# noway/nzcb-circom

Measured on AMD Instinct MI355X. Metric: PLONK proofs/sec for nzcp_live (~2^21 constraints) at 1/2/4/8 MI355X, higher is better.
Workload: dtype u32 limbs: BN254 Fr/Fq Montgomery, 8x32-bit and 9x29-bit (MSM, NTT twiddles, quotient); 1 GPU; nzcp_live fullProve: NZCPPubIdentity(1,351,0,4,2,4) witness on the GPU (600560 signals) + PLONK proof, n=2^21, nPublic=3, 2970 inputs; domain_size=2097152, n_public=3, n_constraints=1785813, n_vars=1782570, n_additions=1182010, proofs_per_gpu=140, total_proofs=140, parallelism=batch-shard x1 (no collective), proofs_in_flight_per_gpu=5

## Files before the change

### nzcb-circom_amd/csrc/msm.h

```cpp
#pragma once
#include <vector>

#include "common.h"
#include "ec.h"
#include "f29.h"

namespace nzcb {

struct MsmBaseTable {
  DevBuf<G1Affine> q;
  size_t n = 0, stride = 0;
  int c = 0, nw = 0;
  bool mont_folded = false;
  bool sparse = false;
  void build(const G1Affine* bases, size_t n, int c, hipStream_t st, bool fold_mont = false);
};

int fixed_base_window();
int lagrange_window();
bool lagrange_sparse();

struct MsmScratch {
  size_t max_points = 0;
  int max_lsets = 1;
  DevBuf<uint32_t> offsets;
  DevBuf<uint32_t> sorted;
  DevBuf<uint32_t> keys_in, keys_out, vals_in;
  DevBuf<uint8_t> sort_tmp;
  size_t sort_tmp_bytes = 0;
  DevBuf<uint32_t> bin_counts, vals_mid;
  DevBuf<uint32_t> lo_seg;
  DevBuf<G1xyzz> buckets;
  DevBuf<G1xyzz> carry_own;
  DevBuf<G1xyzz> carry_cont;
  DevBuf<Xyzz29> buckets29, carry_own29, carry_cont29;
  DevBuf<uint32_t> large;
  DevBuf<uint32_t> large_off;
  DevBuf<Xyzz29> large_part;
  DevBuf<Xyzz29> rowp29, colp29, lines29;
  DevBuf<G1xyzz> seg_tot;
  DevBuf<G1xyzz> seg_run;
  DevBuf<G1xyzz> parts;
  DevBuf<G1xyzz> win;
  G1xyzz* host_win = nullptr;
  uint32_t* host_total = nullptr;
  size_t host_win_cap = 0;
  int cur_c = 0, cur_nsets = 0, cur_nbits = 0, cur_seglen = 0;
  bool cur_fixed = false, cur_sparse = false;
  int cur_a = 0, cur_hb = 0;
  int cur_msets = 1;
  size_t cur_n = 0;
  uint32_t cur_nkeys = 0;
  bool prof = false, prof_phases = false;
  double prof_ms = 0;
  double phase_ms[7] = {0, 0, 0, 0, 0, 0, 0};
  double host_ms = 0;
  double enqueue_ms = 0;
  double sort_host_ms = 0;
  uint64_t prof_launches = 0, prof_points = 0, prof_entries = 0;
  hipEvent_t ev[8] = {nullptr, nullptr, nullptr, nullptr, nullptr, nullptr, nullptr, nullptr};
  hipEvent_t done = nullptr;
  void init(size_t max_points, bool fixed_base = false, int lagrange_sets = 1, bool generic = true);
  ~MsmScratch();
};

int msm_window_bits(size_t n);

void msm_enqueue(MsmScratch& sc, const G1Affine* bases, const Fr* scalars, size_t n, bool scalars_mont,
                 hipStream_t st, const MsmBaseTable* table = nullptr);
G1xyzz msm_finish(MsmScratch& sc, hipStream_t st);
void msm_enqueue_sets(MsmScratch& sc, const Fr* const* scalars, int sets, size_t n, bool scalars_mont,
                      hipStream_t st, const MsmBaseTable* table);
void msm_finish_sets(MsmScratch& sc, hipStream_t st, G1xyzz* out);

inline G1xyzz msm(MsmScratch& sc, const G1Affine* bases, const Fr* scalars, size_t n, bool mont, hipStream_t st,
                  const MsmBaseTable* table = nullptr) {
  msm_enqueue(sc, bases, scalars, n, mont, st, table);
  return msm_finish(sc, st);
}

G1Affine xyzz_to_affine(const G1xyzz& p);

}
```

### nzcb-circom_amd/csrc/msm.hip

```cpp
#include "msm.h"

#include "f29.h"

#include <chrono>
#include <cstdlib>
#include <type_traits>
#include <rocprim/rocprim.hpp>
#include <rocprofiler-sdk-roctx/roctx.h>

namespace nzcb {

static constexpr int kMsmThreads = 256;

#ifndef NZ_TAIL_PRIO
#define NZ_TAIL_PRIO 0
#endif
__device__ __forceinline__ void tail_prio() {
  if constexpr (NZ_TAIL_PRIO > 0) __builtin_amdgcn_s_setprio(NZ_TAIL_PRIO);
}

using SortConfig = rocprim::radix_sort_config<
    rocprim::default_config, rocprim::default_config,
    rocprim::radix_sort_onesweep_config<rocprim::kernel_config<1024, 16>, rocprim::kernel_config<1024, 16>, 10,
                                        rocprim::block_radix_rank_algorithm::match>>;
// ... 17 lines not shown
static constexpr uint32_t kSeqSpan = 64;
static constexpr uint32_t kSeqSpan29 = 16;
static constexpr int kLargeBlocks = 32;
static constexpr int kLargePieceBlocks = 128;
static constexpr int kLargeFinalBlocks = 128;

static constexpr uint32_t kDynThreads = 1u << 18;
static constexpr uint32_t kDynMin = 8;
static constexpr uint32_t kSeqSpanSparse = 3;
static constexpr int kSparsePieceBlocks = 2048;
static constexpr int kSparseFinalBlocks = 512;
__host__ __device__ __forceinline__ uint32_t dyn_chunk(uint32_t m) {
  const uint32_t c = (m + kDynThreads - 1) / kDynThreads;
  return c < kDynMin ? kDynMin : c > kChunk ? kChunk : c;
}
static size_t dyn_threads_bound(size_t entries) {
  const size_t lo = std::min<size_t>(kDynThreads, (entries + kDynMin - 1) / kDynMin);
  return std::max<size_t>(lo, (entries + kChunk - 1) / kChunk);
}

static constexpr int kFbWindow = 20;
int fixed_base_window() {
  static const int c = [] {
    const char* e = std::getenv("NZCB_FB_WINDOW");
    const int v = e ? std::atoi(e) : kFbWindow;
    return (v >= 16 && v <= 20) ? v : kFbWindow;
  }();
  return c;
}

#ifndef NZ_LAGRANGE_WINDOW
#define NZ_LAGRANGE_WINDOW 17
#endif
int lagrange_window() { return NZ_LAGRANGE_WINDOW; }
bool lagrange_sparse() {
  static const bool v = [] {
    const char* e = std::getenv("NZCB_SPARSE");
    return e && std::atoi(e) != 0;
  }();
  return v;
}

int msm_window_bits(size_t n) {
  if (n >= (size_t(1) << 18)) return 16;
  int lg = ilog2(n ? n : 1);
  int c = lg - 3;
  if (c < 4) c = 4;
  if (c > 16) c = 16;
  return c;
}

static inline int num_windows(int c) { return (255 + c - 1) / c; }

template <int C, class F>
__device__ __forceinline__ void for_each_digit(const Fr& s, F&& f) {
  constexpr int NW = (255 + C - 1) / C;
  constexpr uint32_t MASK = (1u << C) - 1u;
  constexpr uint32_t HALF = 1u << (C - 1);
  uint32_t carry = 0;
#pragma unroll
  for (int w = 0; w < NW; w++) {
    const int bit = w * C;
    const int limb = bit >> 5;
    const int sh = bit & 31;
    uint64_t x = s.v[limb];
    if (limb + 1 < 8) x |= (uint64_t)s.v[limb + 1] << 32;
    uint32_t d = ((uint32_t)(x >> sh) & MASK) + carry;
    if (d > HALF) {
      uint32_t mag = (MASK + 1u) - d;
      if (mag) f(w, mag - 1u, 1u);
      carry = 1;
    } else {
      if (d) f(w, d - 1u, 0u);
      carry = 0;
    }
  }
}

#ifdef NZCB_MSM_STATS
template <class F>
static void for_each_digit_host(const Fr& s, int C, F&& f) {
  const int NW = (255 + C - 1) / C;
  const uint32_t MASK = (1u << C) - 1u, HALF = 1u << (C - 1);
  uint32_t carry = 0;
  for (int w = 0; w < NW; w++) {
    const int bit = w * C, limb = bit >> 5, sh = bit & 31;
    uint64_t x = s.v[limb];
    if (limb + 1 < 8) x |= (uint64_t)s.v[limb + 1] << 32;
    uint32_t d = ((uint32_t)(x >> sh) & MASK) + carry;
    if (d > HALF) {
      uint32_t mag = (MASK + 1u) - d;
      if (mag) f(w, mag - 1u, 1u);
      carry = 1;
    } else {
      if (d) f(w, d - 1u, 0u);
      carry = 0;
    }
  }
}
#endif

template <int C>
__global__ void __launch_bounds__(kMsmThreads)
msm_keys_kernel(const Fr* __restrict__ scalars, size_t n, int mont, uint32_t* __restrict__ keys,
                uint32_t* __restrict__ vals) {
  constexpr int NW = (255 + C - 1) / C;
  constexpr uint32_t NB = 1u << (C - 1);
  constexpr uint32_t SENTINEL = NW * NB;
  for (size_t i = (size_t)blockIdx.x * blockDim.x + threadIdx.x; i < n; i += (size_t)gridDim.x * blockDim.x) {
    Fr s = scalars[i];
    if (mont) s = from_mont_fr29(s);
    uint32_t k[NW];
#pragma unroll
    for (int w = 0; w < NW; w++) k[w] = SENTINEL;
    uint32_t sg[NW];
#pragma unroll
    for (int w = 0; w < NW; w++) sg[w] = 0;
    for_each_digit<C>(s, [&](int w, uint32_t b, uint32_t sign) {
      k[w] = (uint32_t)w * NB + b;
      sg[w] = sign << 31;
    });
#pragma unroll
    for (int w = 0; w < NW; w++) {
      keys[(size_t)w * n + i] = k[w];
      vals[(size_t)w * n + i] = (uint32_t)i | sg[w];
    }
  }
}

static constexpr int kBinThreads = 256;
static constexpr int kBinPer = 2;
static constexpr uint32_t kTileScalars = kBinThreads * kBinPer;
static constexpr int kLoThreads = 512;

static constexpr int kDigMont = 1;
static constexpr int kDigMinForm = 2;

__device__ __forceinline__ uint32_t scalar_min_form(Fr& s) {
  constexpr uint32_t H[8] = {0xf8000000u, 0xa1f0fac9u, 0x3cdcb848u, 0x9419f424u,
                             0x40c0ac2eu, 0xdc2822dbu, 0x7098d014u, 0x18322739u};
  bool gt = false, eq = true, lt_r = false, eq_r = true;
#pragma unroll
  for (int l = 7; l >= 0; l--) {
    gt = gt || (eq && s.v[l] > H[l]);
    eq = eq && s.v[l] == H[l];
    lt_r = lt_r || (eq_r && s.v[l] < FrParams::P[l]);
    eq_r = eq_r && s.v[l] == FrParams::P[l];
  }
  if (!(gt && lt_r)) return 0u;
  s = neg(s);
  return 1u;
}

template <int C, int NW>
__device__ __forceinline__ uint32_t bin_entries(const Fr* __restrict__ scalars, size_t i, int mont, size_t stride,
                                                uint32_t (&kk)[NW], uint32_t (&vv)[NW]) {
  Fr s = scalars[i];
  if (mont & kDigMont) s = from_mont_fr29(s);
  const uint32_t flip = (mont & kDigMinForm) ? scalar_min_form(s) : 0u;
  uint32_t live = 0;
#pragma unroll
  for (int w = 0; w < NW; w++) {
    kk[w] = 0;
    vv[w] = 0;
  }
  for_each_digit<C>(s, [&](int w, uint32_t b, uint32_t sign) {
    kk[w] = b;
    vv[w] = (uint32_t)((size_t)w * stride + i) | ((sign ^ flip) << 31);
    live |= 1u << w;
  });
  return live;
}

template <int KB> struct BinKeys {
  static constexpr int LO = KB - 8 > 8 ? KB - 8 : 8;
  using Lo = typename std::conditional<LO <= 8, uint8_t, uint16_t>::type;
  using Full = typename std::conditional<KB <= 16, uint16_t, uint32_t>::type;
};

static constexpr int kMaxSets = 3;
struct BinSets {
  const Fr* p[kMaxSets];
  uint32_t tps;
  uint32_t nb;
};

template <int C, int KB>
__global__ void __launch_bounds__(kBinThreads)
msm_bin_hist_kernel(BinSets sets, size_t n, int mont, uint32_t* __restrict__ counts, uint32_t ntiles) {
  constexpr int NW = (255 + C - 1) / C;
  constexpr int LO = BinKeys<KB>::LO;
  __shared__ uint32_t h[256];
  h[threadIdx.x] = 0;
  __syncthreads();
  const uint32_t set = blockIdx.x / sets.tps, lt = blockIdx.x - set * sets.tps;
  const Fr* __restrict__ scalars = sets.p[set];
  const uint32_t kbase = set * sets.nb;
#pragma unroll
  for (int j = 0; j < kBinPer; j++) {
    const size_t i = (size_t)lt * kTileScalars + (size_t)j * kBinThreads + threadIdx.x;
    if (i < n) {
      uint32_t kk[NW], vv[NW];
      const uint32_t live = bin_entries<C, NW>(scalars, i, mont, 0, kk, vv);
#pragma unroll
      for (int w = 0; w < NW; w++)
        if ((live >> w) & 1u) atomicAdd(&h[(kk[w] + kbase) >> LO], 1u);
    }
  }
  __syncthreads();
  counts[(size_t)threadIdx.x * ntiles + blockIdx.x] = h[threadIdx.x];
}

__device__ __forceinline__ uint32_t wave_incl_scan(uint32_t v) {
  const int lane = threadIdx.x & 63;
#pragma unroll
  for (int off = 1; off < 64; off <<= 1) {
    const uint32_t u = __shfl_up(v, off, 64);
    if (lane >= off) v += u;
  }
  return v;
}

__device__ __forceinline__ uint32_t scan256_excl(uint32_t v, uint32_t* wsum4, uint32_t& total) {
  const uint32_t inc = wave_incl_scan(threadIdx.x < 256 ? v : 0u);
  if (threadIdx.x < 256 && (threadIdx.x & 63) == 63) wsum4[threadIdx.x >> 6] = inc;
  __syncthreads();
  uint32_t off = 0;
  for (int w = 0; w < (int)(threadIdx.x >> 6) && w < 4; w++) off += wsum4[w];
  total = wsum4[0] + wsum4[1] + wsum4[2] + wsum4[3];
  __syncthreads();
  return threadIdx.x < 256 ? off + inc - v : 0u;
}

__global__ void __launch_bounds__(256)
msm_bin_rowscan_kernel(uint32_t* __restrict__ counts, uint32_t ntiles, uint32_t* __restrict__ tail) {
  __shared__ uint32_t wsum[4];
  uint32_t* row = counts + (size_t)blockIdx.x * ntiles;
  uint32_t carry = 0;
  for (uint32_t c0 = 0; c0 < ntiles; c0 += 256) {
    const uint32_t t = c0 + threadIdx.x;
    const uint32_t v = t < ntiles ? row[t] : 0u;
    uint32_t tot;
    const uint32_t ex = scan256_excl(v, wsum, tot);
    if (t < ntiles) row[t] = carry + ex;
    carry += tot;
  }
  if (threadIdx.x == 0) tail[blockIdx.x] = carry;
}

template <int C, int KB>
__global__ void __launch_bounds__(kBinThreads)
msm_bin_scatter_kernel(BinSets sets, size_t n, int mont, size_t stride, const uint32_t* __restrict__ counts,
                       uint32_t ntiles, typename BinKeys<KB>::Lo* __restrict__ lo2, uint32_t* __restrict__ vals2) {
  constexpr int NW = (255 + C - 1) / C;
  constexpr int TE = kTileScalars * NW;
  constexpr int LO = BinKeys<KB>::LO;
  __shared__ uint32_t lcount[256], lstart[256], gbase[256];
  __shared__ uint32_t lval[TE];
  __shared__ typename BinKeys<KB>::Full lkey[TE];
  const uint32_t set = blockIdx.x / sets.tps, lt = blockIdx.x - set * sets.tps;
  const Fr* __restrict__ scalars = sets.p[set];
  const uint32_t kbase = set * sets.nb;
  __shared__ uint32_t wsum[4];
  const uint32_t* tail = counts + (size_t)256 * ntiles;
  {
    uint32_t tot;
    const uint32_t st = scan256_excl(tail[threadIdx.x], wsum, tot);
    gbase[threadIdx.x] = st + counts[(size_t)threadIdx.x * ntiles + blockIdx.x];
    lcount[threadIdx.x] = 0;
  }
  __syncthreads();
  uint32_t kk[kBinPer][NW], vv[kBinPer][NW], rk[kBinPer][NW], live[kBinPer];
#pragma unroll
  for (int j = 0; j < kBinPer; j++) {
    const size_t i = (size_t)lt * kTileScalars + (size_t)j * kBinThreads + threadIdx.x;
    live[j] = 0;
    if (i < n) {
      live[j] = bin_entries<C, NW>(scalars, i, mont, stride, kk[j], vv[j]);
#pragma unroll
      for (int w = 0; w < NW; w++) {
        kk[j][w] += kbase;
        if ((live[j] >> w) & 1u) rk[j][w] = atomicAdd(&lcount[kk[j][w] >> LO], 1u);
      }
    }
  }
  __syncthreads();
  uint32_t total;
  {
    lstart[threadIdx.x] = scan256_excl(lcount[threadIdx.x], wsum, total);
  }
  __syncthreads();
#pragma unroll
  for (int j = 0; j < kBinPer; j++) {
#pragma unroll
    for (int w = 0; w < NW; w++) {
      if ((live[j] >> w) & 1u) {
        const uint32_t q = lstart[kk[j][w] >> LO] + rk[j][w];
        lkey[q] = (typename BinKeys<KB>::Full)kk[j][w];
        lval[q] = vv[j][w];
      }
    }
  }
  __syncthreads();
  for (uint32_t q = threadIdx.x; q < total; q += kBinThreads) {
    const uint32_t key = lkey[q], hb = key >> LO;
    const uint32_t pos = gbase[hb] + (q - lstart[hb]);
    lo2[pos] = (typename BinKeys<KB>::Lo)(key & ((1u << LO) - 1u));
    vals2[pos] = lval[q];
  }
}

template <int NT>
__device__ __forceinline__ uint32_t block_scan_excl(uint32_t* a, uint32_t count, uint32_t* wsum) {
  const uint32_t per = (count + NT - 1) / NT;
  const uint32_t b = threadIdx.x * per;
  uint32_t loc = 0;
  for (uint32_t i = 0; i < per; i++)
    if (b + i < count) loc += a[b + i];
  const uint32_t inc = wave_incl_scan(loc);
  if ((threadIdx.x & 63) == 63) wsum[threadIdx.x >> 6] = inc;
  __syncthreads();
  uint32_t off = 0, tot = 0;
#pragma unroll
  for (int w = 0; w < NT / 64; w++) {
    if (w < (int)(threadIdx.x >> 6)) off += wsum[w];
    tot += wsum[w];
  }
  uint32_t run = off + inc - loc;
  for (uint32_t i = 0; i < per; i++)
    if (b + i < count) {
      const uint32_t v = a[b + i];
      a[b + i] = run;
      run += v;
    }
  __syncthreads();
  return tot;
}

static constexpr uint32_t kLoSeg = 32768;
static constexpr uint32_t kLoU = 8;

__device__ __forceinline__ void lo_regions(const uint32_t* __restrict__ tail, uint32_t* wsum, uint32_t* rs,
                                           uint32_t* rf) {
  const uint32_t t = threadIdx.x;
  const uint32_t cnt = t < 256 ? tail[t] : 0u;
  uint32_t tot, nitems;
  const uint32_t st = scan256_excl(cnt, wsum, tot);
  const uint32_t f = scan256_excl((cnt + kLoSeg - 1) / kLoSeg, wsum, nitems);
  if (t < 256) {
    rs[t] = st;
    rf[t] = f;
  }
  if (t == 0) rf[256] = nitems;
  __syncthreads();
}

__device__ __forceinline__ uint32_t lo_region_of(const uint32_t* rf, uint32_t item) {
  uint32_t lo = 0, hi = 256;
  while (hi - lo > 1) {
    const uint32_t mid = (lo + hi) >> 1;
    if (rf[mid] <= item) lo = mid; else hi = mid;
  }
  return lo;
}

template <int LO>
__global__ void __launch_bounds__(kLoThreads)
msm_lo_count_kernel(const typename std::conditional<LO <= 8, uint8_t, uint16_t>::type* __restrict__ lo2,
                    const uint32_t* __restrict__ counts, uint32_t ntiles, uint32_t* __restrict__ segoff) {
  constexpr uint32_t NL = 1u << LO;
  __shared__ uint32_t h[NL], wsum[kLoThreads / 64], rs[256], rf[257];
  lo_regions(counts + (size_t)256 * ntiles, wsum, rs, rf);
  const uint32_t item = blockIdx.x;
  if (item >= rf[256]) return;
  const uint32_t r = lo_region_of(rf, item);
  const uint32_t* tail = counts + (size_t)256 * ntiles;
  const uint32_t s = rs[r] + (item - rf[r]) * kLoSeg;
  const uint32_t e = min(rs[r] + tail[r], s + kLoSeg);
  for (uint32_t i = threadIdx.x; i < NL; i += kLoThreads) h[i] = 0;
  __syncthreads();
  for (uint32_t p0 = s; p0 < e; p0 += kLoU * kLoThreads) {
    uint32_t k8[kLoU];
#pragma unroll
    for (uint32_t u = 0; u < kLoU; u++) {
      const uint32_t q = p0 + u * kLoThreads + threadIdx.x;
      k8[u] = q < e ? (uint32_t)lo2[q] : NL;
    }
#pragma unroll
    for (uint32_t u = 0; u < kLoU; u++)
      if (k8[u] < NL) atomicAdd(&h[k8[u]], 1u);
  }
  __syncthreads();
  for (uint32_t i = threadIdx.x; i < NL; i += kLoThreads) segoff[(size_t)item * NL + i] = h[i];
}

template <int LO>
__global__ void __launch_bounds__(kLoThreads)
msm_lo_scan_kernel(const uint32_t* __restrict__ counts, uint32_t ntiles, uint32_t* __restrict__ segoff,
                   uint32_t nkeys, uint32_t* __restrict__ offsets, uint32_t* __restrict__ large) {
  constexpr uint32_t NL = 1u << LO;
  __shared__ uint32_t h[NL], wsum[kLoThreads / 64], rs[256], rf[257];
  const uint32_t* tail = counts + (size_t)256 * ntiles;
  lo_regions(tail, wsum, rs, rf);
  const uint32_t hb = blockIdx.x;
  const uint32_t f0 = rf[hb], ns = rf[hb + 1] - f0, s = rs[hb];
  for (uint32_t i = threadIdx.x; i < NL; i += kLoThreads) {
    uint32_t run = 0;
    for (uint32_t g = 0; g < ns; g++) {
      uint32_t* c = segoff + (size_t)(f0 + g) * NL + i;
      const uint32_t v = *c;
      *c = run;
      run += v;
    }
    h[i] = run;
  }
  __syncthreads();
  block_scan_excl<kLoThreads>(h, NL, wsum);
  for (uint32_t i = threadIdx.x; i < NL; i += kLoThreads) {
    const uint32_t base = s + h[i];
    const uint32_t key = (hb << LO) | i;
    if (key < nkeys) offsets[key] = base;
    for (uint32_t g = 0; g < ns; g++) segoff[(size_t)(f0 + g) * NL + i] += base;
  }
  if (hb == 255 && threadIdx.x == 0) offsets[nkeys] = s + tail[255];
  if (hb == 0 && threadIdx.x == 0) large[0] = 0;
}

template <int LO, int NT = kLoThreads, uint32_t U = kLoU>
__global__ void __launch_bounds__(NT)
msm_lo_scatter_kernel(const typename std::conditional<LO <= 8, uint8_t, uint16_t>::type* __restrict__ lo2,
                      const uint32_t* __restrict__ vals2, const uint32_t* __restrict__ counts, uint32_t ntiles,
                      const uint32_t* __restrict__ segoff, uint32_t* __restrict__ sorted) {
  using Lo = typename std::conditional<LO <= 8, uint8_t, uint16_t>::type;
  constexpr uint32_t NL = 1u << LO;
  constexpr uint32_t kLoThreads = NT, kLoU = U;
  __shared__ uint32_t h[NL], lcnt[NL], lst[NL];
  __shared__ uint32_t wsum[kLoThreads / 64], rs[256], rf[257];
  __shared__ uint32_t lv[kLoU * kLoThreads];
  __shared__ Lo lk[kLoU * kLoThreads];
  lo_regions(counts + (size_t)256 * ntiles, wsum, rs, rf);
  const uint32_t item = blockIdx.x;
  if (item >= rf[256]) return;
  const uint32_t r = lo_region_of(rf, item);
  const uint32_t* tail = counts + (size_t)256 * ntiles;
  const uint32_t s = rs[r] + (item - rf[r]) * kLoSeg;
  const uint32_t e = min(rs[r] + tail[r], s + kLoSeg);
  for (uint32_t i = threadIdx.x; i < NL; i += kLoThreads) h[i] = segoff[(size_t)item * NL + i];
  for (uint32_t p0 = s; p0 < e; p0 += kLoU * kLoThreads) {
    uint32_t k8[kLoU], v8[kLoU], r8[kLoU];
    for (uint32_t i = threadIdx.x; i < NL; i += kLoThreads) lcnt[i] = 0;
    __syncthreads();
#pragma unroll
// ... 663 lines not shown
    if (s == 0 && blockIdx.y == 0 && total_out) host_put(total_out, *entries);
    host_put_done();
  }
}

__global__ void __launch_bounds__(kMsmThreads)
msm_table_kernel(const G1Affine* __restrict__ bases, size_t n, size_t stride, int c, int nw, Fq k261, int fold,
                 Fr kinv, G1Affine* __restrict__ q) {
  const size_t i = (size_t)blockIdx.x * blockDim.x + threadIdx.x;
  if (i >= n) return;
  const G1Affine P = bases[i];
  if (P.is_inf()) {
    for (int w = 0; w < nw; w++) q[(size_t)w * stride + i] = P;
    return;
  }
  G1xyzz acc = xyzz_from_affine(P);
  if (fold) {
    acc = G1xyzz::inf();
    for (int b = 253; b >= 0; b--) {
      acc = xyzz_dbl(acc);
      if ((kinv.v[b >> 5] >> (b & 31)) & 1u) acc = xyzz_add_affine(acc, P.x, P.y);
    }
  }
  for (int w = 0; w < nw; w++) {
    if (w)
      for (int k = 0; k < c; k++) acc = xyzz_dbl(acc);
    const Fq ti = inverse(acc.ZZ * acc.ZZZ);
    G1Affine r;
    r.x = acc.X * (acc.ZZZ * ti) * k261;
    r.y = acc.Y * (acc.ZZ * ti) * k261;
    q[(size_t)w * stride + i] = r;
  }
}

void MsmBaseTable::build(const G1Affine* bases, size_t npts, int cbits, hipStream_t st, bool fold_mont) {
  n = npts;
  mont_folded = fold_mont;
  stride = npts;
  c = cbits;
  nw = num_windows(c);
  if ((size_t)nw * stride >= (size_t(1) << 31)) throw Error(NZCB_ERR_ARG, "msm table too large for 31-bit indices");
  q.alloc((size_t)nw * stride);
  Fq thirty_two = Fq::zero();
  thirty_two.v[0] = 32;
  const Fq k261 = to_mont(thirty_two);
  Fr one_raw = Fr::zero();
  one_raw.v[0] = 1;
  const Fr kinv = from_mont(one_raw);
  hipLaunchKernelGGL(msm_table_kernel, dim3(grid_for(n, kMsmThreads, 1u << 30)), dim3(kMsmThreads), 0, st, bases, n,
                     stride, c, nw, k261, fold_mont ? 1 : 0, kinv, q.p);
  NZ_HIP(hipGetLastError());
}

static void lmark(const char* what) {
  static const bool on = std::getenv("NZCB_MARK_LAUNCHES") != nullptr;
  if (on) roctxMarkA(what);
}

static size_t lo_items_bound(size_t entries) { return 256 + entries / kLoSeg + 1; }

struct MsmPlan {
  int c, nw, nsets, seglen, nseg, nbits, nslots, nparts;
  int lb, a, hb, ltiles, htiles;
  int msets;
  uint32_t nb, nkeys;
  size_t entries;
};

static MsmPlan make_plan(size_t n, const MsmBaseTable* t, int msets = 1) {
  MsmPlan p;
  p.c = t ? t->c : msm_window_bits(n);
  p.nw = num_windows(p.c);
  p.nsets = t ? 1 : p.nw;
  p.msets = t ? msets : 1;
  p.nb = 1u << (p.c - 1);
  p.nkeys = p.nb * (uint32_t)p.nsets * (uint32_t)p.msets;
  p.seglen = (int)(p.nb < (uint32_t)kSegLen ? p.nb : kSegLen);
  p.nseg = (int)(p.nb / p.seglen);
  p.nbits = 0;
  while ((1 << p.nbits) < p.nseg) p.nbits++;
  p.nslots = p.nbits + 1;
  p.nparts = (p.nseg + kSumThreads * kSumPer - 1) / (kSumThreads * kSumPer);
  p.lb = p.c - 1;
  p.a = (p.lb + 1) / 2;
  p.hb = p.lb - p.a;
  p.ltiles = (1 << p.a) / kTileSide;
  p.htiles = (1 << p.hb) / kTileSide;
  p.entries = n * (size_t)p.nw * (size_t)p.msets;
  return p;
}

void MsmScratch::init(size_t maxp, bool fixed_base, int lagrange_sets, bool generic) {
  if (lagrange_sets < 1 || lagrange_sets > kMaxSets) throw Error(NZCB_ERR_ARG, "msm scratch: 1..3 Lagrange sets");
  if (!fixed_base) generic = true;
  max_points = maxp;
  max_lsets = lagrange_sets;
  size_t max_entries = 0, max_keys = 0, max_seg = 0, max_slots = 0, max_parts = 0, max_tiles = 0, max_lines = 0;
  auto fit = [&](const MsmPlan& p) {
    max_entries = std::max(max_entries, p.entries);
    max_keys = std::max(max_keys, (size_t)p.nkeys);
    if (p.nsets == 1) {
      max_slots = std::max(max_slots, (size_t)(p.lb + 1) * p.msets);
      max_tiles = std::max(max_tiles, (size_t)p.nb / kTileSide * p.msets);
      max_lines = std::max(max_lines, (((size_t)1 << p.hb) + ((size_t)1 << p.a)) * p.msets);
    } else {
      max_seg = std::max(max_seg, (size_t)p.nseg * p.nsets);
      max_slots = std::max(max_slots, (size_t)p.nslots * p.nsets);
      max_parts = std::max(max_parts, (size_t)p.nslots * p.nsets * p.nparts);
    }
  };
  for (size_t n = 1;; n <<= 1) {
    size_t m = n < maxp ? n : maxp;
    fit(make_plan(m, nullptr));
    if (m == maxp) break;
  }
  MsmPlan fp{};
  if (fixed_base) {
    MsmBaseTable t;
    t.c = fixed_base_window();
    fp = make_plan(maxp, &t);
    fit(fp);
    t.c = lagrange_window();
    const MsmPlan lp = make_plan(maxp, &t, lagrange_sets);
    fit(lp);
    if (lp.entries > fp.entries) fp = lp;
  }
  const size_t ge = generic ? max_entries : 1;
  offsets.alloc(max_keys + 1);
  sorted.alloc(max_entries);
  keys_in.alloc(ge);
  keys_out.alloc(max_entries);
  vals_in.alloc(ge);
  sort_tmp_bytes = 0;
  if (generic) {
    radix_sort(nullptr, sort_tmp_bytes, keys_in.p, keys_out.p, vals_in.p, sorted.p, max_entries, 21, nullptr);
  }
  sort_tmp.alloc(sort_tmp_bytes + 16);
  const size_t nthreads = std::max((max_entries + kChunk - 1) / kChunk, dyn_threads_bound(max_entries)) + 1;
  buckets.alloc(generic ? max_keys : 1);
  carry_own.alloc(generic ? nthreads : 1);
  carry_cont.alloc(generic ? nthreads : 1);
  large.alloc(max_keys + 1);
  if (fixed_base) {
    buckets29.alloc(max_keys);
    large_off.alloc(max_keys + 2);
    large_part.alloc(nthreads / kPieceCarries + max_keys + 1);
    carry_own29.alloc(nthreads);
    carry_cont29.alloc(nthreads);
    rowp29.alloc(max_tiles);
    colp29.alloc(max_tiles);
    lines29.alloc(max_lines);
    bin_counts.alloc((size_t)256 * ((maxp + kTileScalars - 1) / kTileScalars) * lagrange_sets + 256);
    vals_mid.alloc(max_entries);
    lo_seg.alloc(lo_items_bound(max_entries) * ((size_t)1 << BinKeys<19>::LO));
  }
  seg_tot.alloc(max_seg && generic ? max_seg : 1);
  seg_run.alloc(max_seg && generic ? max_seg : 1);
  parts.alloc(max_parts && generic ? max_parts : 1);
  win.alloc(max_slots);
  host_win_cap = max_slots;
  NZ_HIP(hipHostMalloc((void**)&host_win, (max_slots + 1) * sizeof(G1xyzz), hipHostMallocCoherent));
  host_total = (uint32_t*)(host_win + max_slots);
}

MsmScratch::~MsmScratch() {
  if (host_win) (void)hipHostFree(host_win);
  if (done) (void)hipEventDestroy(done);
  for (auto& e : ev)
    if (e) (void)hipEventDestroy(e);
}

static void keys_dispatch(int c, const Fr* scalars, size_t n, int mont, MsmScratch& sc, hipStream_t st) {
  auto launch = [&](auto cc) {
    constexpr int C = decltype(cc)::value;
    hipLaunchKernelGGL(msm_keys_kernel<C>, dim3(grid_for(n, kMsmThreads, 1u << 30)), dim3(kMsmThreads), 0, st,
                       scalars, n, mont, sc.keys_in.p, sc.vals_in.p);
  };
  switch (c) {
#define NZ_CASE(K) case K: launch(std::integral_constant<int, K>()); break;
    NZ_CASE(4) NZ_CASE(5) NZ_CASE(6) NZ_CASE(7) NZ_CASE(8) NZ_CASE(9) NZ_CASE(10) NZ_CASE(11) NZ_CASE(12)
    NZ_CASE(13) NZ_CASE(14) NZ_CASE(15) NZ_CASE(16)
#undef NZ_CASE
    default: throw Error(NZCB_ERR_INTERNAL, "bad msm window");
  }
  NZ_HIP(hipGetLastError());
}

G1Affine xyzz_to_affine(const G1xyzz& p) {
  G1Affine r;
  if (p.is_inf()) {
    r.x = Fq::zero();
    r.y = Fq::zero();
    return r;
  }
  r.x = p.X * inverse(p.ZZ);
  r.y = p.Y * inverse(p.ZZZ);
  return r;
}

template <class Mark>
static void fixed_bucketing(MsmScratch& sc, const MsmPlan& p, const BinSets& sets, size_t n, int mdig,
                            const MsmBaseTable* table, hipStream_t st, const Mark& mark) {
  const uint32_t tps = (uint32_t)((n + kTileScalars - 1) / kTileScalars);
  const uint32_t ntiles = tps * (uint32_t)p.msets;
  BinSets bs = sets;
  bs.tps = tps;
  bs.nb = p.nb;
  uint32_t* tail = sc.bin_counts.p + (size_t)256 * ntiles;
  auto run_bins = [&](auto cc, auto kb) {
    constexpr int C = decltype(cc)::value;
    constexpr int KB = decltype(kb)::value;
    using Lo = typename BinKeys<KB>::Lo;
    constexpr int LO = BinKeys<KB>::LO;
    Lo* lo2 = (Lo*)sc.keys_out.p;
    hipLaunchKernelGGL((msm_bin_hist_kernel<C, KB>), dim3(ntiles), dim3(kBinThreads), 0, st, bs, n, mdig,
                       sc.bin_counts.p, ntiles);
    NZ_HIP(hipGetLastError());
    lmark("mark: L hist");
    mark(1);
    hipLaunchKernelGGL(msm_bin_rowscan_kernel, dim3(256), dim3(256), 0, st, sc.bin_counts.p, ntiles, tail);
    lmark("mark: L rowscan");
    hipLaunchKernelGGL((msm_bin_scatter_kernel<C, KB>), dim3(ntiles), dim3(kBinThreads), 0, st, bs, n, mdig,
                       table->stride, sc.bin_counts.p, ntiles, lo2, sc.vals_mid.p);
    NZ_HIP(hipGetLastError());
    lmark("mark: L scatter");
    mark(2);
    const dim3 igrid((unsigned)lo_items_bound(p.entries));
    hipLaunchKernelGGL(msm_lo_count_kernel<LO>, igrid, dim3(kLoThreads), 0, st, (const Lo*)lo2, sc.bin_counts.p,
                       ntiles, sc.lo_seg.p);
    NZ_HIP(hipGetLastError());
    lmark("mark: L lo_count");
    hipLaunchKernelGGL(msm_lo_scan_kernel<LO>, dim3(256), dim3(kLoThreads), 0, st, sc.bin_counts.p, ntiles,
                       sc.lo_seg.p, p.nkeys, sc.offsets.p, sc.large.p);
    NZ_HIP(hipGetLastError());
    lmark("mark: L lo_scan");
    constexpr int sNT = LO > 8 ? 1024 : kLoThreads;
    constexpr uint32_t sU = LO > 8 ? 16 : kLoU;
    hipLaunchKernelGGL((msm_lo_scatter_kernel<LO, sNT, sU>), igrid, dim3(sNT), 0, st, (const Lo*)lo2, sc.vals_mid.p,
                       sc.bin_counts.p, ntiles, (const uint32_t*)sc.lo_seg.p, sc.sorted.p);
    NZ_HIP(hipGetLastError());
    lmark("mark: L lo_scatter");
  };
  using std::integral_constant;
  if (p.msets > 1) {
    if (p.c != 17) throw Error(NZCB_ERR_INTERNAL, "msm sets: the Lagrange window (17) only");
    run_bins(integral_constant<int, 17>(), integral_constant<int, 18>());
    return;
  }
  switch (p.c) {
    case 16: run_bins(integral_constant<int, 16>(), integral_constant<int, 15>()); break;
    case 17: run_bins(integral_constant<int, 17>(), integral_constant<int, 16>()); break;
    case 18: run_bins(integral_constant<int, 18>(), integral_constant<int, 17>()); break;
    case 19: run_bins(integral_constant<int, 19>(), integral_constant<int, 18>()); break;
    case 20: run_bins(integral_constant<int, 20>(), integral_constant<int, 19>()); break;
    default: throw Error(NZCB_ERR_INTERNAL, "bad fixed-base msm window");
  }
}

static void msm_enqueue_impl(MsmScratch& sc, const G1Affine* bases, const Fr* const* scalars, int msets, size_t n,
                             bool mont, hipStream_t st, const MsmBaseTable* table) {
  const auto t_enq = std::chrono::steady_clock::now();
  struct EnqueueClock {
    MsmScratch& sc;
    std::chrono::steady_clock::time_point t0;
    ~EnqueueClock() {
      if (sc.prof && sc.prof_phases)
        sc.enqueue_ms += std::chrono::duration<double, std::milli>(std::chrono::steady_clock::now() - t0).count();
    }
  } enqueue_clock{sc, t_enq};
  if (msets < 1 || msets > kMaxSets || (msets > 1 && (!table || msets > sc.max_lsets)))
    throw Error(NZCB_ERR_ARG, "msm sets: 1..3 over a table, within the scratch's sizing");
  sc.cur_n = n;
  sc.cur_msets = table ? msets : 1;
  if (n == 0) return;
  if (!sc.done) NZ_HIP(hipEventCreateWithFlags(&sc.done, hipEventDisableTiming));
  if (n > sc.max_points) throw Error(NZCB_ERR_ARG, "msm larger than scratch");
  if (table && n > table->n) throw Error(NZCB_ERR_ARG, "msm larger than its base table");
  if (table && table->mont_folded && !mont) throw Error(NZCB_ERR_ARG, "2^-256-folded table needs Montgomery scalars");
  if (table && (!sc.buckets29.p || !sc.bin_counts.p))
    throw Error(NZCB_ERR_ARG, "msm scratch was not sized for the fixed-base schedule");
  const int mdig = (mont && !(table && table->mont_folded)) ? 1 : 0;
  const MsmPlan p = make_plan(n, table, msets);
#ifdef NZCB_MSM_STATS
  if (table && !table->mont_folded) {
    NZ_HIP(hipStreamSynchronize(st));
    for (int k = 0; k < msets; k++) {
      std::vector<Fr> h(n);
      NZ_HIP(hipMemcpy(h.data(), scalars[k], n * sizeof(Fr), hipMemcpyDeviceToHost));
      size_t e_pos = 0, e_min = 0, nneg = 0, zero = 0, hist[17] = {0};
      for (size_t i = 0; i < n; i++) {
        Fr v = mdig ? from_mont(h[i]) : h[i];
        if (v.is_zero()) { zero++; continue; }
        const Fr w = neg(v);
        auto digits = [&](const Fr& x) {
          size_t d = 0;
          for_each_digit_host(x, p.c, [&](int, uint32_t, uint32_t) { d++; });
          return d;
        };
        const size_t dp = digits(v), dn = digits(w);
        e_pos += dp;
        e_min += dp <= dn ? dp : dn;
        if (dn < dp) nneg++;
        const size_t dm = dp <= dn ? dp : dn;
        hist[dm < 16 ? dm : 16]++;
      }
      fprintf(stderr, "MSMSCALARS set=%d n=%zu c=%d zero=%zu entries=%zu entries_minform=%zu flipped=%zu hist_minform=",
              k, n, p.c, zero, e_pos, e_min, nneg);
      for (int b = 0; b < 17; b++) fprintf(stderr, "%zu%c", hist[b], b == 16 ? '\n' : ',');
    }
  }
#endif
  if (p.entries > sc.sorted.n || p.nkeys + 1 > sc.offsets.n)
    throw Error(NZCB_ERR_ARG, "msm scratch was not sized for this schedule");
  if (table && ((size_t)p.nb / kTileSide * msets > sc.rowp29.n ||
                (((size_t)1 << p.hb) + ((size_t)1 << p.a)) * msets > sc.lines29.n ||
                (size_t)(p.lb + 1) * msets > sc.host_win_cap || (msets > 1 && p.c >= kStripMinC)))
    throw Error(NZCB_ERR_ARG, "msm scratch was not sized for this window");
  sc.cur_c = p.c;
  sc.cur_nsets = p.nsets;
  sc.cur_nbits = p.nbits;
  sc.cur_seglen = p.seglen;
  sc.cur_nkeys = p.nkeys;
  sc.cur_fixed = table != nullptr;
  sc.cur_a = p.a;
  sc.cur_hb = p.hb;
  sc.cur_msets = p.msets;
  const bool phases = sc.prof && sc.prof_phases;
  if (sc.prof && !sc.ev[0])
    for (auto& e : sc.ev) NZ_HIP(hipEventCreate(&e));
  auto mark = [&](int i) {
    if (phases) NZ_HIP(hipEventRecord(sc.ev[i], st));
  };
  mark(0);
  if (table) {
    BinSets bs{};
    for (int k = 0; k < msets; k++) bs.p[k] = scalars[k];
    fixed_bucketing(sc, p, bs, n, mdig | (table->mont_folded ? 0 : kDigMinForm), table, st, mark);
  } else {
    keys_dispatch(p.c, scalars[0], n, mdig, sc, st);
    mark(1);
    size_t tmp = sc.sort_tmp_bytes;
    int end_bit = 1;
    while ((1u << end_bit) <= p.nkeys) end_bit++;
    const auto t_sort = std::chrono::steady_clock::now();
    radix_sort(sc.sort_tmp.p, tmp, sc.keys_in.p, sc.keys_out.p, sc.vals_in.p, sc.sorted.p, p.entries, end_bit, st);
    if (phases)
      sc.sort_host_ms += std::chrono::duration<double, std::milli>(std::chrono::steady_clock::now() - t_sort).count();
    mark(2);
    hipLaunchKernelGGL(msm_offsets_kernel, dim3(grid_for((size_t)p.nkeys + 1, kMsmThreads, 1u << 30)),
                       dim3(kMsmThreads), 0, st, sc.keys_out.p, p.entries, p.nkeys, sc.offsets.p);
    NZ_HIP(hipGetLastError());
  }
  if (sc.prof) NZ_HIP(hipEventRecord(sc.ev[3], st));
  const bool sparse = table && table->sparse;
  sc.cur_sparse = sparse;
  const uint32_t chunk = sparse ? 0u : chunk_for(p.entries);
  const size_t nthreads = sparse ? dyn_threads_bound(p.entries) : (p.entries + chunk - 1) / chunk;
  const dim3 agrid(grid_for(nthreads, kMsmThreads, 1u << 30));
  const G1Affine* gather = table ? table->q.p : bases;
  if (table) {
    if (chunk == kChunk || sparse)
      hipLaunchKernelGGL(msm_accumulate29_kernel<true>, agrid, dim3(kMsmThreads), 0, st, chunk, gather, sc.sorted.p,
                         sc.offsets.p, p.nkeys, nthreads, sc.buckets29.p, sc.carry_own29.p, sc.carry_cont29.p);
    else
      hipLaunchKernelGGL(msm_accumulate29_kernel<false>, agrid, dim3(kMsmThreads), 0, st, chunk, gather, sc.sorted.p,
                         sc.offsets.p, p.nkeys, nthreads, sc.buckets29.p, sc.carry_own29.p, sc.carry_cont29.p);
  } else {
    hipLaunchKernelGGL(msm_accumulate_kernel, agrid, dim3(kMsmThreads), 0, st, chunk, gather, sc.sorted.p, sc.offsets.p,
                       p.nkeys, nthreads, sc.buckets.p, sc.carry_own.p, sc.carry_cont.p);
  }
  NZ_HIP(hipGetLastError());
  lmark("mark: L accumulate");
  if (sc.prof) NZ_HIP(hipEventRecord(sc.ev[4], st));
  const dim3 fgrid(grid_for(p.nkeys, kMsmThreads, 1u << 30));
  if (table) {
    hipLaunchKernelGGL(msm_finalize29_kernel, fgrid, dim3(kMsmThreads), 0, st, chunk, sc.offsets.p, p.nkeys,
// ... 188 lines not shown
```

Before: 48.02 proofs/s.

## Record decoded scalar digits in histogram pass and reuse them in scatter

The histogram kernel now stores each scalar's signed digits (key+1 with a sign bit) in a new scratch buffer. The scatter kernel reads these records instead of reloading scalars and redoing Montgomery conversion, min-form negation and digit decomposition. Small scalars that fit in a single digit get a short record, so the scatter reads one word instead of NW. The cost is extra scratch memory plus the global traffic of writing and reading the record. The histogram loop is also no longer unrolled.

```diff
diff --git a/nzcb-circom_amd/csrc/msm.h b/nzcb-circom_amd/csrc/msm.h
--- a/nzcb-circom_amd/csrc/msm.h
+++ b/nzcb-circom_amd/csrc/msm.h
@@ -29,6 +29,7 @@
   DevBuf<uint8_t> sort_tmp;
   size_t sort_tmp_bytes = 0;
   DevBuf<uint32_t> bin_counts, vals_mid;
+  DevBuf<uint32_t> bin_rec;
   DevBuf<uint32_t> lo_seg;
   DevBuf<G1xyzz> buckets;
   DevBuf<G1xyzz> carry_own;
diff --git a/nzcb-circom_amd/csrc/msm.hip b/nzcb-circom_amd/csrc/msm.hip
--- a/nzcb-circom_amd/csrc/msm.hip
+++ b/nzcb-circom_amd/csrc/msm.hip
@@ -193,24 +193,45 @@
   return 1u;
 }
 
+static constexpr uint32_t kRecShort = 1u << 30;
+static constexpr uint32_t kRecSign = 1u << 31;
+static constexpr uint32_t kRecKey = kRecShort - 1u;
+
 template <int C, int NW>
-__device__ __forceinline__ uint32_t bin_entries(const Fr* __restrict__ scalars, size_t i, int mont, size_t stride,
-                                                uint32_t (&kk)[NW], uint32_t (&vv)[NW]) {
+__device__ __forceinline__ void digit_words(const Fr& s, uint32_t flip, uint32_t (&r)[NW]) {
+#pragma unroll
+  for (int w = 0; w < NW; w++) r[w] = 0;
+  for_each_digit<C>(s, [&](int w, uint32_t b, uint32_t sign) { r[w] = (b + 1u) | ((sign ^ flip) << 31); });
+}
+
+template <int C, int NW, int LO>
+__device__ __forceinline__ void bin_decode(const Fr* __restrict__ scalars, size_t i, int mont, uint32_t kbase,
+                                           uint32_t* h, uint32_t* __restrict__ rec, size_t recn) {
   Fr s = scalars[i];
   if (mont & kDigMont) s = from_mont_fr29(s);
-  const uint32_t flip = (mont & kDigMinForm) ? scalar_min_form(s) : 0u;
-  uint32_t live = 0;
-#pragma unroll
-  for (int w = 0; w < NW; w++) {
-    kk[w] = 0;
-    vv[w] = 0;
-  }
-  for_each_digit<C>(s, [&](int w, uint32_t b, uint32_t sign) {
-    kk[w] = b;
-    vv[w] = (uint32_t)((size_t)w * stride + i) | ((sign ^ flip) << 31);
-    live |= 1u << w;
-  });
-  return live;
+  uint32_t flip = 0;
+  bool small = false;
+  if (mont & kDigMinForm) {
+    flip = scalar_min_form(s);
+    small = rec && (s.v[1] | s.v[2] | s.v[3] | s.v[4] | s.v[5] | s.v[6] | s.v[7]) == 0u && s.v[0] < (1u << (C - 1));
+  }
+  if (small) {
+    const uint32_t d = s.v[0];
+    if (d) atomicAdd(&h[(d - 1u + kbase) >> LO], 1u);
+    rec[0] = kRecShort | (d ? d | (flip << 31) : 0u);
+  } else {
+    uint32_t r[NW];
+#pragma unroll
+    for (int w = 0; w < NW; w++) r[w] = 0;
+    for_each_digit<C>(s, [&](int w, uint32_t b, uint32_t sign) {
+      atomicAdd(&h[(b + kbase) >> LO], 1u);
+      r[w] = (b + 1u) | ((sign ^ flip) << 31);
+    });
+    if (rec) {
+#pragma unroll
+      for (int w = 0; w < NW; w++) rec[(size_t)w * recn] = r[w];
+    }
+  }
 }
 
 template <int KB> struct BinKeys {
@@ -228,7 +249,8 @@
 
 template <int C, int KB>
 __global__ void __launch_bounds__(kBinThreads)
-msm_bin_hist_kernel(BinSets sets, size_t n, int mont, uint32_t* __restrict__ counts, uint32_t ntiles) {
+msm_bin_hist_kernel(BinSets sets, size_t n, int mont, uint32_t* __restrict__ counts, uint32_t ntiles,
+                    uint32_t* __restrict__ rec) {
   constexpr int NW = (255 + C - 1) / C;
   constexpr int LO = BinKeys<KB>::LO;
   __shared__ uint32_t h[256];
@@ -237,16 +259,14 @@
   const uint32_t set = blockIdx.x / sets.tps, lt = blockIdx.x - set * sets.tps;
   const Fr* __restrict__ scalars = sets.p[set];
   const uint32_t kbase = set * sets.nb;
-#pragma unroll
+  const size_t recn = (size_t)ntiles * kTileScalars;
+#pragma unroll 1
   for (int j = 0; j < kBinPer; j++) {
-    const size_t i = (size_t)lt * kTileScalars + (size_t)j * kBinThreads + threadIdx.x;
-    if (i < n) {
-      uint32_t kk[NW], vv[NW];
-      const uint32_t live = bin_entries<C, NW>(scalars, i, mont, 0, kk, vv);
-#pragma unroll
-      for (int w = 0; w < NW; w++)
-        if ((live >> w) & 1u) atomicAdd(&h[(kk[w] + kbase) >> LO], 1u);
-    }
+    const uint32_t slot = (uint32_t)j * kBinThreads + threadIdx.x;
+    const size_t i = (size_t)lt * kTileScalars + slot;
+    if (i < n)
+      bin_decode<C, NW, LO>(scalars, i, mont, kbase, h, rec ? rec + (size_t)blockIdx.x * kTileScalars + slot : nullptr,
+                            recn);
   }
   __syncthreads();
   counts[(size_t)threadIdx.x * ntiles + blockIdx.x] = h[threadIdx.x];
@@ -291,8 +311,9 @@
 
 template <int C, int KB>
 __global__ void __launch_bounds__(kBinThreads)
-msm_bin_scatter_kernel(BinSets sets, size_t n, int mont, size_t stride, const uint32_t* __restrict__ counts,
-                       uint32_t ntiles, typename BinKeys<KB>::Lo* __restrict__ lo2, uint32_t* __restrict__ vals2) {
+msm_bin_scatter_kernel(BinSets sets, size_t n, size_t stride, const uint32_t* __restrict__ counts, uint32_t ntiles,
+                       const uint32_t* __restrict__ rec, typename BinKeys<KB>::Lo* __restrict__ lo2,
+                       uint32_t* __restrict__ vals2) {
   constexpr int NW = (255 + C - 1) / C;
   constexpr int TE = kTileScalars * NW;
   constexpr int LO = BinKeys<KB>::LO;
@@ -302,6 +323,7 @@
   const uint32_t set = blockIdx.x / sets.tps, lt = blockIdx.x - set * sets.tps;
   const Fr* __restrict__ scalars = sets.p[set];
   const uint32_t kbase = set * sets.nb;
+  const size_t recn = (size_t)ntiles * kTileScalars;
   __shared__ uint32_t wsum[4];
   const uint32_t* tail = counts + (size_t)256 * ntiles;
   {
@@ -311,17 +333,28 @@
     lcount[threadIdx.x] = 0;
   }
   __syncthreads();
-  uint32_t kk[kBinPer][NW], vv[kBinPer][NW], rk[kBinPer][NW], live[kBinPer];
+  uint32_t rw[kBinPer][NW], rk[kBinPer][NW];
 #pragma unroll
   for (int j = 0; j < kBinPer; j++) {
-    const size_t i = (size_t)lt * kTileScalars + (size_t)j * kBinThreads + threadIdx.x;
-    live[j] = 0;
+    const uint32_t slot = (uint32_t)j * kBinThreads + threadIdx.x;
+    const size_t i = (size_t)lt * kTileScalars + slot;
+#pragma unroll
+    for (int w = 0; w < NW; w++) rw[j][w] = 0;
     if (i < n) {
-      live[j] = bin_entries<C, NW>(scalars, i, mont, stride, kk[j], vv[j]);
+      if (rec) {
+        const uint32_t* __restrict__ r = rec + (size_t)blockIdx.x * kTileScalars + slot;
+        rw[j][0] = r[0];
+        if (!(rw[j][0] & kRecShort)) {
+#pragma unroll
+          for (int w = 1; w < NW; w++) rw[j][w] = r[(size_t)w * recn];
+        }
+      } else {
+        digit_words<C, NW>(scalars[i], 0u, rw[j]);
+      }
 #pragma unroll
       for (int w = 0; w < NW; w++) {
-        kk[j][w] += kbase;
-        if ((live[j] >> w) & 1u) rk[j][w] = atomicAdd(&lcount[kk[j][w] >> LO], 1u);
+        const uint32_t f = rw[j][w] & kRecKey;
+        if (f) rk[j][w] = atomicAdd(&lcount[(f - 1u + kbase) >> LO], 1u);
       }
     }
   }
@@ -333,12 +366,15 @@
   __syncthreads();
 #pragma unroll
   for (int j = 0; j < kBinPer; j++) {
+    const uint32_t i = lt * kTileScalars + (uint32_t)j * kBinThreads + threadIdx.x;
 #pragma unroll
     for (int w = 0; w < NW; w++) {
-      if ((live[j] >> w) & 1u) {
-        const uint32_t q = lstart[kk[j][w] >> LO] + rk[j][w];
-        lkey[q] = (typename BinKeys<KB>::Full)kk[j][w];
-        lval[q] = vv[j][w];
+      const uint32_t f = rw[j][w] & kRecKey;
+      if (f) {
+        const uint32_t key = f - 1u + kbase;
+        const uint32_t q = lstart[key >> LO] + rk[j][w];
+        lkey[q] = (typename BinKeys<KB>::Full)key;
+        lval[q] = ((uint32_t)w * (uint32_t)stride + i) | (rw[j][w] & kRecSign);
       }
     }
   }
@@ -1308,6 +1344,8 @@
     lines29.alloc(max_lines);
     bin_counts.alloc((size_t)256 * ((maxp + kTileScalars - 1) / kTileScalars) * lagrange_sets + 256);
     vals_mid.alloc(max_entries);
+    bin_rec.alloc((maxp + kTileScalars - 1) / kTileScalars * kTileScalars *
+                  (size_t)std::max(num_windows(16), num_windows(lagrange_window()) * lagrange_sets));
     lo_seg.alloc(lo_items_bound(max_entries) * ((size_t)1 << BinKeys<19>::LO));
   }
   seg_tot.alloc(max_seg && generic ? max_seg : 1);
@@ -1369,15 +1407,19 @@
     using Lo = typename BinKeys<KB>::Lo;
     constexpr int LO = BinKeys<KB>::LO;
     Lo* lo2 = (Lo*)sc.keys_out.p;
+    uint32_t* rec = (mdig & kDigMinForm) ? sc.bin_rec.p : nullptr;
+    if (!rec && mdig != 0) throw Error(NZCB_ERR_INTERNAL, "msm bucketing: converted scalars need the digit record");
+    if (rec && (size_t)ntiles * kTileScalars * num_windows(C) > sc.bin_rec.n)
+      throw Error(NZCB_ERR_ARG, "msm scratch was not sized for this window's digit record");
     hipLaunchKernelGGL((msm_bin_hist_kernel<C, KB>), dim3(ntiles), dim3(kBinThreads), 0, st, bs, n, mdig,
-                       sc.bin_counts.p, ntiles);
+                       sc.bin_counts.p, ntiles, rec);
     NZ_HIP(hipGetLastError());
     lmark("mark: L hist");
     mark(1);
     hipLaunchKernelGGL(msm_bin_rowscan_kernel, dim3(256), dim3(256), 0, st, sc.bin_counts.p, ntiles, tail);
     lmark("mark: L rowscan");
-    hipLaunchKernelGGL((msm_bin_scatter_kernel<C, KB>), dim3(ntiles), dim3(kBinThreads), 0, st, bs, n, mdig,
-                       table->stride, sc.bin_counts.p, ntiles, lo2, sc.vals_mid.p);
+    hipLaunchKernelGGL((msm_bin_scatter_kernel<C, KB>), dim3(ntiles), dim3(kBinThreads), 0, st, bs, n,
+                       table->stride, sc.bin_counts.p, ntiles, (const uint32_t*)rec, lo2, sc.vals_mid.p);
     NZ_HIP(hipGetLastError());
     lmark("mark: L scatter");
     mark(2);
```

Result: no change. 48.25 proofs/s, median of 5 (+0.5%).
